# lh3/miniasm

Measured on NVIDIA H100. Metric: paf_overlaps_per_sec_ingest_to_gfa, higher is better.
Workload: dtype int64/uint32 (+3 float32 predicates)

## Files before the change

miniasm_b200/csrc/ingest_dev.cu:

```cuda
#include "ingest_dev.cuh"
#include "shard_comm.cuh"
#include <cub/cub.cuh>

struct PLine {
	uint32_t ql, qs, qe, tl, ts, te, ml_rev, bl;
	uint32_t tdelta;
	uint32_t qnl, tnl;
	uint32_t nf;
};

struct __align__(16) PRec {
	uint32_t qs, qe, ts, te;
	uint32_t ml_rev;
	uint32_t bl_f;
	uint32_t slot_q, slot_t;
};
static_assert(sizeof(PRec) == 32, "PRec layout");
constexpr uint32_t NOSLOT = 0xffffffffu;

constexpr int NL_THREADS = 256;
constexpr int NL_PER_THREAD = 4;
constexpr uint64_t NL_TILE = (uint64_t)NL_THREADS * NL_PER_THREAD * 16;

__device__ __forceinline__ uint32_t nl_mask4(uint32_t w) { return __vcmpeq4(w, 0x0a0a0a0au); }

__device__ __forceinline__ uint32_t nl_bits16(const char *text, size_t len, uint64_t off)
{
	if (off >= len) return 0;
	uint32_t bits = 0;
	if (off + 16 <= len) {
		const uint4 w = __ldg(reinterpret_cast<const uint4*>(text + off));
		const uint32_t m[4] = { nl_mask4(w.x), nl_mask4(w.y), nl_mask4(w.z), nl_mask4(w.w) };
		#pragma unroll
		for (int k = 0; k < 4; ++k) bits |= ((m[k] & 1) | (m[k] >> 7 & 2) | (m[k] >> 14 & 4) | (m[k] >> 21 & 8)) << (4 * k);
	} else for (uint64_t k = 0; off + k < len; ++k) bits |= (uint32_t)(text[off + k] == '\n') << k;
	if (off + 16 >= len && len - 1 - off < 16) bits &= ~(1u << (len - 1 - off));
	return bits;
}

__global__ void __launch_bounds__(NL_THREADS) k_nl_count(const char *__restrict__ text, size_t len, uint64_t n_tile, uint64_t *cnt)
{
	typedef cub::BlockReduce<uint32_t, NL_THREADS> BR;
	__shared__ typename BR::TempStorage ts;
	for (uint64_t t = blockIdx.x; t < n_tile; t += gridDim.x) {
		uint32_t c = 0;
		#pragma unroll
		for (int k = 0; k < NL_PER_THREAD; ++k) c += __popc(nl_bits16(text, len, t * NL_TILE + ((uint64_t)k * NL_THREADS + threadIdx.x) * 16));
		c = BR(ts).Sum(c);
		if (threadIdx.x == 0) cnt[t] = c;
		__syncthreads();
	}
	if (blockIdx.x == 0 && threadIdx.x == 0) cnt[n_tile] = 0;
}

__global__ void __launch_bounds__(NL_THREADS) k_nl_write(const char *__restrict__ text, size_t len, uint64_t n_tile, const uint64_t *__restrict__ base, uint64_t *out)
{
	typedef cub::BlockScan<uint32_t, NL_THREADS> BS;
	__shared__ typename BS::TempStorage ts;
	for (uint64_t t = blockIdx.x; t < n_tile; t += gridDim.x) {
		uint64_t at = base[t];
		#pragma unroll
		for (int k = 0; k < NL_PER_THREAD; ++k) {
			const uint64_t off = t * NL_TILE + ((uint64_t)k * NL_THREADS + threadIdx.x) * 16;
			uint32_t bits = nl_bits16(text, len, off), rank, total;
			BS(ts).ExclusiveSum((uint32_t)__popc(bits), rank, total);
			uint64_t *o = out + at + rank;
			while (bits) { const int b = __ffs(bits) - 1; *o++ = off + b + 1; bits &= bits - 1; }
			at += total;
			__syncthreads();
		}
	}
}

__host__ __device__ __forceinline__ uint32_t field_to_u32(const char *p, const char *e)
{
	while (p < e && (*p == ' ' || (*p >= '\t' && *p <= '\r'))) ++p;
	bool neg = false;
	if (p < e && (*p == '-' || *p == '+')) neg = *p == '-', ++p;
	while (p < e && *p == '0') ++p;
	unsigned long long v = 0;
	int nd = 0;
	for (; p < e; ++p, ++nd) {
		const unsigned dgt = (unsigned)(*p - '0');
		if (dgt > 9) break;
		if (nd < 18) { v = v * 10 + dgt; continue; }
// ... 33 lines not shown
{
	const uint32_t len = (uint32_t)(e - p);
	uint32_t nt = 0;
	{
		const uintptr_t a = (uintptr_t)p & ~(uintptr_t)3;
		const int lead = (int)((uintptr_t)p - a);
		for (int off = -lead; off < (int)len && nt < 11; off += 4) {
			uint32_t bits = tab_bits4(*reinterpret_cast<const uint32_t*>(p + off));
			while (bits) {
#ifdef __CUDA_ARCH__
				const int pos = off + __ffs(bits) - 1;
#else
				const int pos = off + __builtin_ctz(bits);
#endif
				bits &= bits - 1;
				if (pos >= 0 && pos < (int)len && nt < 11) tab[nt++ * 32] = (uint32_t)pos;
			}
		}
	}
	const uint32_t nf = nt + 1 < 11 ? nt + 1 : 11;
	#define COL_S(k) ((k) ? tab[((k) - 1) * 32] + 1 : 0u)
	#define COL_T(k) ((uint32_t)(k) < nt ? tab[(k) * 32] : len)
	memset(&r, 0, sizeof(r));
	r.nf = nf;
	r.qnl = COL_T(0);
	if (nf > 1) r.ql = num_field(p, COL_S(1), COL_T(1));
	if (nf > 2) r.qs = num_field(p, COL_S(2), COL_T(2));
	if (nf > 3) r.qe = num_field(p, COL_S(3), COL_T(3));
	if (nf > 4) { const uint32_t s4 = COL_S(4); r.ml_rev = (COL_T(4) > s4 && p[s4] == '-') ? 0x80000000u : 0; }
	if (nf > 5) {
		const uint32_t s5 = COL_S(5), t5 = COL_T(5);
		r.tnl = t5 - s5, r.tdelta = s5;
	}
	if (nf > 6) r.tl = num_field(p, COL_S(6), COL_T(6));
	if (nf > 7) r.ts = num_field(p, COL_S(7), COL_T(7));
	if (nf > 8) r.te = num_field(p, COL_S(8), COL_T(8));
	if (nf > 9) r.ml_rev |= num_field(p, COL_S(9), COL_T(9)) & 0x7fffffffu;
	if (nf > 10) r.bl = num_field(p, COL_S(10), COL_T(10));
	#undef COL_S
	#undef COL_T
}

struct NameTab {
	unsigned long long *key;
	unsigned long long *first;
	uint32_t *id;
	uint64_t mask;
	uint32_t *hits = nullptr;
};
constexpr int NT_OFF_BITS = 37;
constexpr unsigned long long NT_OFF_MASK = (1ull << NT_OFF_BITS) - 1;

__device__ __forceinline__ uint32_t tab_insert(const NameTab &t, const char *__restrict__ text, const char *nm, uint32_t nl, uint64_t goff, uint64_t occ,
                                               unsigned long long *overflow)
{
	const uint64_t h = name_hash(nm, 0, nl, 0);
	const unsigned long long mine = (h >> 37) << NT_OFF_BITS | (goff + 1);
	uint64_t s = h & t.mask;
	for (int probe = 0; probe < 1 << 14; ++probe, s = (s + 1) & t.mask) {
		unsigned long long k = t.key[s];
		if (k == 0) {
			k = atomicCAS(&t.key[s], 0ull, mine);
			if (k == 0) k = mine;
		}
		if ((k ^ mine) >> NT_OFF_BITS) continue;
		bool same = k == mine;
		if (!same) {
			const char *w = text + ((k & NT_OFF_MASK) - 1);
			same = true;
			for (uint32_t i = 0; same && i < nl; ++i) same = w[i] == nm[i];
			same = same && w[nl] == '\t';
		}
		if (!same) continue;
		if (t.first[s] > occ) atomicMin(&t.first[s], (unsigned long long)occ);
		return (uint32_t)s;
	}
	atomicAdd(overflow, 1ull);
	return 0;
}

constexpr int PT_THREADS = 128;
constexpr uint32_t PT_TILE = 8192;
constexpr uint32_t PT_OVER = 1024;
constexpr uint32_t PT_LIST = 1024;
static_assert(PT_TILE == PT_THREADS * 64, "each thread scans 64 bytes of its tile for line starts");
static_assert(PT_OVER % 16 == 0 && PT_OVER <= PT_TILE, "the overhang ends inside the tile after the parsed ones");

typedef cub::ScanTileState<unsigned long long> LineTileState;
typedef cub::TilePrefixCallbackOp<unsigned long long, ::cuda::std::plus<unsigned long long>, LineTileState> LinePrefixOp;

enum { PC_PARSED = 0, PC_STORED, PC_OVERFLOW, PC_LINES, PC_CUT, PC_N };

__device__ __forceinline__ uint32_t nl_bits_u4(const uint4 w)
{
	const uint32_t m[4] = { nl_mask4(w.x), nl_mask4(w.y), nl_mask4(w.z), nl_mask4(w.w) };
	uint32_t bits = 0;
	#pragma unroll
	for (int k = 0; k < 4; ++k) bits |= ((m[k] & 1) | (m[k] >> 7 & 2) | (m[k] >> 14 & 4) | (m[k] >> 21 & 8)) << (4 * k);
	return bits;
}

__global__ void k_tiles_init(LineTileState ts, int n_tile) { ts.InitializeStatus(n_tile); }

template <class P>
__global__ void __launch_bounds__(PT_THREADS)
k_parse_tiles(const char *__restrict__ text, size_t len, size_t avail, uint64_t t_lo, uint64_t line_cap, unsigned *tile_ctr, LineTileState tstate,
              int min_span, int min_match, int bi_dir, P pol)
{
	typedef cub::BlockScan<uint32_t, PT_THREADS> BS;
	__shared__ __align__(16) char s_text[PT_TILE + PT_OVER + 16];
	__shared__ uint16_t s_start[PT_LIST + 1];
	__shared__ uint32_t s_vals[PT_THREADS / 32][11][32];
	__shared__ typename BS::TempStorage s_scan;
	__shared__ typename LinePrefixOp::TempStorage s_pref;
	__shared__ unsigned long long s_first, s_tile, s_eol;
	__shared__ uint32_t s_nl;
	const uint32_t lane = threadIdx.x & 31;
	if (threadIdx.x == 0) s_tile = t_lo + atomicAdd(tile_ctr, 1u), s_nl = ~0u;
	__syncthreads();
	const uint64_t t = s_tile, b0 = t * PT_TILE, b1 = b0 + PT_TILE < len ? b0 + PT_TILE : len;
	const uint64_t w_end = b1 + PT_OVER < avail ? b1 + PT_OVER : avail;
	{
		const uint32_t n16 = (uint32_t)((w_end - b0 + 15) >> 4);
		for (uint32_t k = threadIdx.x; k < n16; k += PT_THREADS)
			reinterpret_cast<uint4*>(s_text)[k] = __ldg(reinterpret_cast<const uint4*>(text + b0) + k);
	}
	__syncthreads();
	const uint32_t my0 = threadIdx.x * 64, lim = (uint32_t)((b1 == len ? len - 1 : b1) - b0);
	uint64_t bits = 0;
	#pragma unroll
	for (int k = 0; k < 4; ++k) bits |= (uint64_t)nl_bits_u4(reinterpret_cast<const uint4*>(s_text + my0)[k]) << (16 * k);
	bits &= lim <= my0 ? 0ull : lim - my0 >= 64 ? ~0ull : (1ull << (lim - my0)) - 1;
	const bool line0 = t == 0 && threadIdx.x == 0;
	uint32_t rank, n;
	BS(s_scan).ExclusiveSum((uint32_t)__popcll(bits) + line0, rank, n);
	for (uint32_t o = lim + threadIdx.x; o < (uint32_t)(w_end - b0); o += PT_THREADS)
		if (s_text[o] == '\n' && b0 + o < len) { atomicMin(&s_nl, o); break; }
	if (threadIdx.x < 32) {
		if (t == 0) {
			if (threadIdx.x == 0) tstate.SetInclusive(0, n), s_first = 0;
		} else {
			LinePrefixOp op(tstate, s_pref, ::cuda::std::plus<unsigned long long>(), (int)t);
			const unsigned long long ex = op(n);
			if (threadIdx.x == 0) s_first = ex;
		}
	}
	__syncthreads();
	const uint64_t first = pol.line_base() + s_first;
	if (threadIdx.x == 0 && b1 == len) pol.lines_end(first + n);
	if (n == 0) return;
	uint64_t last_eol = s_nl != ~0u ? b0 + s_nl : w_end >= len ? len : ~0ull;
	if (last_eol == ~0ull) {
		if (threadIdx.x < 32) {
			uint64_t e = ~0ull;
			for (uint64_t p = w_end; p < avail; p += 32 * 16) {
				const uint64_t q = p + 16 * lane;
				uint32_t m = 0;
				for (uint32_t k = 0; k < 16 && q + k < avail; ++k) m |= (uint32_t)(text[q + k] == '\n') << k;
				const unsigned hit = __ballot_sync(0xffffffffu, m != 0);
				if (hit) { e = __shfl_sync(0xffffffffu, q + __ffs(m) - 1, __ffs(hit) - 1); break; }
			}
			if (e == ~0ull && avail == len) e = len;
			if (threadIdx.x == 0) {
				s_eol = e;
				if (e == ~0ull) pol.cut();
			}
		}
		__syncthreads();
		last_eol = s_eol;
	}
	unsigned n_parsed = 0, n_pass = 0;
	for (uint32_t r0 = 0; r0 < n; r0 += PT_LIST) {
		{
			uint32_t r = rank;
			uint64_t b = bits;
			if (line0) { if (r == r0) s_start[0] = 0; ++r; }
			for (; b && r <= r0 + PT_LIST; ++r, b &= b - 1)
				if (r >= r0) s_start[r - r0] = (uint16_t)(my0 + __ffsll((long long)b));
		}
		__syncthreads();
		const uint32_t cnt = n - r0 < PT_LIST ? n - r0 : PT_LIST;
		for (uint32_t j0 = 0; j0 < cnt; j0 += PT_THREADS) {
			const uint32_t j = j0 + threadIdx.x;
			const uint64_t i = first + r0 + j;
			uint32_t sq = NOSLOT, st = 0;
			if (j < cnt && i < line_cap) {
				const uint64_t s = b0 + s_start[j];
				uint64_t eol = r0 + j + 1 < n ? b0 + s_start[j + 1] - 1 : last_eol;
				if (eol != ~0ull) {
					const char *base = eol <= w_end ? s_text - b0 : text;
					if (eol - s > 1 && base[eol - 1] == '\r') --eol;
					PLine r;
					parse_line(base + s, base + eol, r, &s_vals[threadIdx.x >> 5][0][lane]);
					bool stored = false;
					if (r.nf >= 10) {
						++n_parsed;
						stored = !(r.qe - r.qs < (uint32_t)min_span || r.te - r.ts < (uint32_t)min_span || (int)(r.ml_rev & 0x7fffffffu) < min_match);
						n_pass += stored;
					}
					pol.line(text, base, s, i, r, stored, bi_dir, sq, st);
				}
			}
			if (uint32_t *hits = pol.hits()) {
				const unsigned grp = __match_any_sync(0xffffffffu, sq);
				if (sq != NOSLOT && lane == (uint32_t)__ffs(grp) - 1) atomicAdd(&hits[sq], (uint32_t)__popc(grp));
				if (sq != NOSLOT && bi_dir && st != sq) atomicAdd(&hits[st], 1u);
			}
		}
		__syncthreads();
	}
	pol.flush(lane, __reduce_add_sync(0xffffffffu, n_parsed), __reduce_add_sync(0xffffffffu, n_pass));
}

struct ParseStore {
	NameTab tab;
	PRec *out;
	uint64_t *start;
	unsigned long long *counts;

	__device__ __forceinline__ uint64_t line_base() const { return 0; }
	__device__ __forceinline__ void lines_end(uint64_t n) const { counts[PC_LINES] = n; }
	__device__ __forceinline__ void cut() const { atomicAdd(counts + PC_CUT, 1ull); }
	__device__ __forceinline__ uint32_t *hits() const { return tab.hits; }
	__device__ __forceinline__ void line(const char *text, const char *base, uint64_t s, uint64_t i, const PLine &r, bool stored, int, uint32_t &sq, uint32_t &st)
	{
		if (stored) {
			sq = tab_insert(tab, text, base + s, r.qnl, s, 2 * i, counts + PC_OVERFLOW);
			st = tab_insert(tab, text, base + s + r.tdelta, r.tnl, s + r.tdelta, 2 * i + 1, counts + PC_OVERFLOW);
		}
		start[i] = s;
		*reinterpret_cast<uint4*>(out + i) = make_uint4(r.qs, r.qe, r.ts, r.te);
		*(reinterpret_cast<uint4*>(out + i) + 1) = make_uint4(r.ml_rev, (r.bl & 0x7fffffffu) | (r.nf >= 11 ? 0x80000000u : 0u), sq, st);
	}
	__device__ __forceinline__ void flush(uint32_t lane, unsigned n_parsed, unsigned n_pass) const
	{
		if (lane == 0) {
			if (n_parsed) atomicAdd(counts + PC_PARSED, (unsigned long long)n_parsed);
			if (n_pass) atomicAdd(counts + PC_STORED, (unsigned long long)n_pass);
		}
	}
};

__device__ __forceinline__ uint32_t line_bl(const PRec *ln, uint64_t i, uint32_t carry_bl)
{
	if (ln[i].bl_f >> 31) return ln[i].bl_f & 0x7fffffffu;
	for (uint64_t j = i; j-- > 0;)
		if (ln[j].bl_f >> 31) return ln[j].bl_f & 0x7fffffffu;
	return carry_bl & 0x7fffffffu;
}

struct SlotUsed {
	const unsigned long long *first;
	__device__ __forceinline__ bool operator()(uint64_t s) const { return first[s] != ~0ull; }
};

__device__ __forceinline__ void occ_name(const char *text, const uint64_t *start, uint64_t occ, uint64_t *noff, uint32_t *nlen, uint32_t *slen)
{
	const char *p = text + start[occ >> 1];
	uint64_t q = 0;
	if (occ & 1) { int tabs = 0; while (tabs < 5) tabs += p[q++] == '\t'; }
	uint64_t e = q;
	while (p[e] != '\t') ++e;
	*noff = start[occ >> 1] + q, *nlen = (uint32_t)(e - q);
	uint64_t f = e + 1;
	while (p[f] != '\t') ++f;
	*slen = field_to_u32(p + e + 1, p + f);
}

__global__ void k_nocont_mark(const PRec *ln, uint64_t n_lines, const char *text, const uint64_t *start, int max_hang, float int_frac, uint8_t *excl)
{
	for (uint64_t i = blockIdx.x * (uint64_t)blockDim.x + threadIdx.x; i < n_lines; i += (uint64_t)gridDim.x * blockDim.x) {
		const PRec r = ln[i];
		if (r.slot_q == NOSLOT) continue;
		uint64_t no; uint32_t nl, ql, tl;
		occ_name(text, start, 2 * i, &no, &nl, &ql);
		occ_name(text, start, 2 * i + 1, &no, &nl, &tl);
		const bool rev = r.ml_rev >> 31;
		const int l5 = (int)(rev ? tl - r.te : r.ts), l3 = (int)(rev ? r.ts : tl - r.te);
		if (ql >> 1 > tl) {
			if (l5 > max_hang >> 2 || l3 > max_hang >> 2 || (float)(r.te - r.ts) < __fmul_rn((float)tl, int_frac)) continue;
			if ((int)r.qs - l5 > max_hang << 1 && (int)(ql - r.qe) - l3 > max_hang << 1) excl[r.slot_t] = 1;
		} else if (ql < tl >> 1) {
			if (r.qs > (uint32_t)(max_hang >> 2) || ql - r.qe > (uint32_t)(max_hang >> 2) || (float)(r.qe - r.qs) < __fmul_rn((float)ql, int_frac)) continue;
			if (l5 - (int)r.qs > max_hang << 1 && l3 - (int)(ql - r.qe) > max_hang << 1) excl[r.slot_q] = 1;
		}
	}
}

__global__ void k_nocont_drop(PRec *ln, uint64_t n_lines, const uint8_t *excl, int bi_dir, NameTab t)
{
	for (uint64_t i = blockIdx.x * (uint64_t)blockDim.x + threadIdx.x; i < n_lines; i += (uint64_t)gridDim.x * blockDim.x) {
		const uint32_t sq = ln[i].slot_q, st = ln[i].slot_t;
		if (sq == NOSLOT) continue;
// ... 126 lines not shown
	void *tmp = d.tmp(tb);
	cub::DeviceRadixSort::SortPairs(tmp, tb, dk, dv, (int)n, lo_bit, hi_bit, d.stream);
	++d.n_lib;
	d.zero_scal(SC_AUX, 1);
	rank(dk.Current(), dv.Current(), n, d.d_scal + SC_AUX);
	const unsigned long long tot_len = d.get_scal(SC_AUX);
	d.free(fa); d.free(fb); d.free(sb);
	return tot_len;
}

template <class Rank>
static void rank_reads(MabDev &d, const NameTab &tab, uint64_t cap, int lo_bit, int hi_bit, Rank rank, DHits &h, DNames &names, IngestStats &st,
                       uint32_t *&cur, uint32_t *&bfirst)
{
	uint64_t *slots = mab_alloc<uint64_t>(d, cap);
	const uint32_t n_seq = names_alloc(d, names, list_slots(d, cap, SlotUsed{tab.first}, slots));
	uint32_t *read_cnt = mab_alloc<uint32_t>(d, (size_t)n_seq + 1), *first = mab_alloc<uint32_t>(d, (size_t)n_seq + 1);
	MAB_CUDA(cudaMemsetAsync(read_cnt + n_seq, 0, 4, d.stream));
	st.tot_len = rank_slots(d, slots, n_seq, tab.first, lo_bit, hi_bit,
	                        [&](const unsigned long long *fs, const uint64_t *ss, uint32_t n, unsigned long long *tot) { rank(fs, ss, n, tot, read_cnt); });
	d.free(slots);
	d.trace("ingest:rank_ids");
	dh_bucket_first(d, read_cnt, n_seq, first);
	MAB_CUDA(cudaMemsetAsync(read_cnt, 0, (size_t)n_seq * 4, d.stream));
	uint32_t n_hits;
	MAB_CUDA(cudaMemcpyAsync(&n_hits, first + n_seq, 4, cudaMemcpyDeviceToHost, d.stream));
	d.sync();
	dh_reserve(d, h, n_hits ? n_hits : 1);
	h.n = n_hits, h.n_seq = n_seq;
	st.n_hits = n_hits, st.n_seq = n_seq;
	cur = read_cnt, bfirst = first;
}

static NameTab tab_alloc(MabDev &d, uint64_t cap, bool with_hits)
{
	NameTab tab;
	tab.key = (unsigned long long*)mab_alloc<uint64_t>(d, cap);
	tab.first = (unsigned long long*)mab_alloc<uint64_t>(d, cap);
	tab.id = mab_alloc<uint32_t>(d, cap);
	tab.mask = cap - 1;
	MAB_CUDA(cudaMemsetAsync(tab.key, 0, cap * 8, d.stream));
	MAB_CUDA(cudaMemsetAsync(tab.first, 0xff, cap * 8, d.stream));
	if (with_hits) {
		tab.hits = mab_alloc<uint32_t>(d, cap);
		MAB_CUDA(cudaMemsetAsync(tab.hits, 0, cap * 4, d.stream));
	}
	return tab;
}

static void tab_free(MabDev &d, NameTab &t)
{
	d.free(t.key); d.free(t.first); d.free(t.id);
	if (t.hits) d.free(t.hits);
	t = NameTab{nullptr, nullptr, nullptr, 0};
}

struct Parsed {
	uint64_t *start = nullptr;
	PRec *ln = nullptr;
	NameTab tab{nullptr, nullptr, nullptr, 0};
	uint64_t cap = 0, n_lines = 0, n_parsed = 0;
	uint32_t regrow = 0;
};

static inline uint64_t line_estimate(size_t len) { return len / 24 + 1024; }
static inline uint64_t tab_cap_for(uint64_t line_cap) { uint64_t cap = 1ull << 20; while (cap < line_cap / 8) cap <<= 1; return cap; }

static LineTileState tiles_alloc(MabDev &d, uint64_t n_tile, void **mem)
{
	if (n_tile >= (1ull << 31) - 64) { fprintf(stderr, "[E::miniasm_b200] more than 2^31 tiles of PAF on one GPU\n"); exit(73); }
	size_t bytes = 0;
	MAB_CUDA(LineTileState::AllocationSize((int)n_tile, bytes));
	*mem = d.alloc(bytes);
	LineTileState ts;
	MAB_CUDA(ts.Init((int)n_tile, *mem, bytes));
	return ts;
}

static void tiles_reset(MabDev &d, LineTileState ts, uint64_t n_tile)
{
	MAB_LAUNCH(d, k_tiles_init, mab_grid(n_tile, 256, 1u << 30), 256, 0, ts, (int)n_tile);
}

static void parse_resident(MabDev &d, const char *d_text, size_t len, int min_span, int min_match, int bi_dir, bool count_hits, Parsed &p)
{
	const uint64_t n_tile = (len + PT_TILE - 1) / PT_TILE;
	uint64_t line_cap = line_estimate(len), cap = tab_cap_for(line_cap);
	unsigned *ctr = mab_alloc<unsigned>(d, 1);
	void *ts_mem = nullptr;
	const LineTileState ts = tiles_alloc(d, n_tile, &ts_mem);
	for (;;) {
		p.start = mab_alloc<uint64_t>(d, line_cap);
		p.ln = mab_alloc<PRec>(d, line_cap);
		p.tab = tab_alloc(d, cap, count_hits);
		d.zero_scal(SC_COUNT, PC_N);
		if (n_tile) {
			tiles_reset(d, ts, n_tile);
			MAB_CUDA(cudaMemsetAsync(ctr, 0, 4, d.stream));
			MAB_LAUNCH(d, k_parse_tiles<ParseStore>, (unsigned)n_tile, PT_THREADS, 0, d_text, len, len, 0, line_cap, ctr, ts, min_span, min_match, bi_dir,
			           ParseStore{p.tab, p.ln, p.start, d.d_scal + SC_COUNT});
		}
		p.n_parsed = d.get_scal(SC_COUNT + PC_PARSED);
		p.n_lines = d.h_scal[SC_COUNT + PC_LINES];
		const bool more_lines = p.n_lines > line_cap, overflow = d.h_scal[SC_COUNT + PC_OVERFLOW] != 0;
		if (!more_lines && !overflow) break;
		d.free(p.start); d.free(p.ln); tab_free(d, p.tab);
		if (more_lines) line_cap = p.n_lines;
		if (overflow) cap <<= 2, ++p.regrow;
		if (cap > (1ull << 33)) { fprintf(stderr, "[E::miniasm_b200] read-name table overflow\n"); exit(77); }
	}
	d.free(ctr); d.free(ts_mem);
	p.cap = cap;
}

static void ingest_finish(MabDev &d, const char *d_text, size_t len, uint64_t *start, PRec *ln, uint64_t n_lines, NameTab tab, uint64_t cap, int bi_dir,
                          const NoContParams *nocont, DHits &h, DNames &names, IngestStats &st);

void ingest_paf(MabDev &d, const char *d_text, size_t len, int min_span, int min_match, int bi_dir, DHits &h, DNames &names, IngestStats &st,
                const NoContParams *nocont)
{
	ingest_open(len, h, names, st);
	if (len == 0) { dh_reserve(d, h, 1); return; }

	d.trace("ingest:begin");
	Parsed p;
	parse_resident(d, d_text, len, min_span, min_match, bi_dir, true, p);
	st.n_parsed = p.n_parsed, st.n_lines = p.n_lines, st.name_regrow = p.regrow;
	d.trace("ingest:parse");
	ingest_finish(d, d_text, len, p.start, p.ln, p.n_lines, p.tab, p.cap, bi_dir, nocont, h, names, st);
}

static bool stream_parse(MabDev &d, char *d_text, const char *host_text, size_t len, int min_span, int min_match, int bi_dir, bool count_hits, Parsed &p)
{
	const uint64_t CH_TILES = (64ull << 20) / PT_TILE, n_tile = (len + PT_TILE - 1) / PT_TILE;
	const uint64_t n_chunk = (n_tile + CH_TILES - 1) / CH_TILES;
	const uint64_t line_cap = line_estimate(len), cap = tab_cap_for(line_cap);
	p.start = mab_alloc<uint64_t>(d, line_cap);
	p.ln = mab_alloc<PRec>(d, line_cap);
	p.tab = tab_alloc(d, cap, count_hits);
	unsigned *ctr = mab_alloc<unsigned>(d, n_chunk);
	MAB_CUDA(cudaMemsetAsync(ctr, 0, n_chunk * 4, d.stream));
	void *ts_mem = nullptr;
	const LineTileState ts = tiles_alloc(d, n_tile, &ts_mem);
	tiles_reset(d, ts, n_tile);
	d.zero_scal(SC_COUNT, PC_N);
	if (!d.copy_stream) MAB_CUDA(cudaStreamCreateWithFlags(&d.copy_stream, cudaStreamNonBlocking));
	std::vector<cudaEvent_t> ev(n_chunk);
	cudaEvent_t ready;
	MAB_CUDA(cudaEventCreateWithFlags(&ready, cudaEventDisableTiming));
	MAB_CUDA(cudaEventRecord(ready, d.stream));
	MAB_CUDA(cudaStreamWaitEvent(d.copy_stream, ready, 0));
	uint64_t t_done = 0;
	for (uint64_t k = 0; k < n_chunk; ++k) {
		const uint64_t t0 = k * CH_TILES, t1 = (k + 1) * CH_TILES < n_tile ? (k + 1) * CH_TILES : n_tile;
		const uint64_t b0 = t0 * PT_TILE, b1 = t1 * PT_TILE < len ? t1 * PT_TILE : len;
		MAB_CUDA(cudaEventCreateWithFlags(&ev[k], cudaEventDisableTiming));
		MAB_CUDA(cudaMemcpyAsync(d_text + b0, host_text + b0, b1 - b0, cudaMemcpyHostToDevice, d.copy_stream));
		MAB_CUDA(cudaEventRecord(ev[k], d.copy_stream));
		MAB_CUDA(cudaStreamWaitEvent(d.stream, ev[k], 0));
		const uint64_t t_hi = k + 1 == n_chunk ? n_tile : t1 - 1;
		MAB_LAUNCH(d, k_parse_tiles<ParseStore>, (unsigned)(t_hi - t_done), PT_THREADS, 0, d_text, len, b1, t_done, line_cap, ctr + k, ts, min_span, min_match,
		           bi_dir, ParseStore{p.tab, p.ln, p.start, d.d_scal + SC_COUNT});
		t_done = t_hi;
	}
	p.n_parsed = d.get_scal(SC_COUNT + PC_PARSED);
	for (uint64_t k = 0; k < n_chunk; ++k) MAB_CUDA(cudaEventDestroy(ev[k]));
	MAB_CUDA(cudaEventDestroy(ready));
	d.free(ctr); d.free(ts_mem);
	p.n_lines = d.h_scal[SC_COUNT + PC_LINES];
	if (p.n_lines > line_cap || d.h_scal[SC_COUNT + PC_OVERFLOW] != 0 || d.h_scal[SC_COUNT + PC_CUT] != 0) {
		d.free(p.start); d.free(p.ln); tab_free(d, p.tab);
		p = Parsed();
		return false;
	}
	p.cap = cap;
	return true;
}

void ingest_paf_stream(MabDev &d, char *d_text, const char *host_text, size_t len, int min_span, int min_match, int bi_dir,
                       DHits &h, DNames &names, IngestStats &st)
{
	ingest_open(len, h, names, st);
	if (len == 0) { dh_reserve(d, h, 1); return; }
	Parsed p;
	if (!stream_parse(d, d_text, host_text, len, min_span, min_match, bi_dir, true, p)) {
		ingest_paf(d, d_text, len, min_span, min_match, bi_dir, h, names, st, nullptr);
		++st.name_regrow;
		return;
	}
	st.n_parsed = p.n_parsed, st.n_lines = p.n_lines;
	d.trace("ingest:stream (copy + parse + dictionary + hit counts)");
	ingest_finish(d, d_text, len, p.start, p.ln, p.n_lines, p.tab, p.cap, bi_dir, nullptr, h, names, st);
}

static void ingest_finish(MabDev &d, const char *d_text, size_t len, uint64_t *start, PRec *ln, uint64_t n_lines, NameTab tab, uint64_t cap, int bi_dir,
                          const NoContParams *nocont, DHits &h, DNames &names, IngestStats &st)
{
	if (2 * n_lines >= (1ull << 32)) { fprintf(stderr, "[E::miniasm_b200] more than 2^31 PAF lines on one GPU\n"); exit(73); }
	d.trace("ingest:dictionary");
	if (nocont) {
		uint8_t *excl = mab_alloc<uint8_t>(d, cap);
		MAB_CUDA(cudaMemsetAsync(excl, 0, cap, d.stream));
		MAB_LAUNCH(d, k_nocont_mark, mab_grid(n_lines, 256), 256, 0, ln, n_lines, d_text, start, nocont->max_hang, nocont->int_frac, excl);
		d.zero_scal(SC_AUX, 1);
		MAB_LAUNCH(d, k_count_u8, mab_grid(cap, 256), 256, 0, excl, cap, d.d_scal + SC_AUX);
		MAB_CUDA(cudaMemsetAsync(tab.first, 0xff, cap * 8, d.stream));
		MAB_CUDA(cudaMemsetAsync(tab.hits, 0, cap * 4, d.stream));
		MAB_LAUNCH(d, k_nocont_drop, mab_grid(n_lines, 256), 256, 0, ln, n_lines, excl, bi_dir, tab);
		st.n_dropped = d.get_scal(SC_AUX);
		d.free(excl);
		d.trace("ingest:-R prefilter");
	}
	uint32_t *read_cnt, *first;
	rank_reads(d, tab, cap, 0, (int)bits_for(2 * n_lines + 1), [&](const unsigned long long *fs, const uint64_t *ss, uint32_t n, unsigned long long *tot, uint32_t *cnt) {
		MAB_LAUNCH(d, k_dict_rank, mab_grid(n, 256), 256, 0, fs, ss, n, tab, d_text, start, names.off, names.nlen, names.slen, tot, cnt);
	}, h, names, st, read_cnt, first);
	if (h.n) MAB_LAUNCH(d, k_hit_emit, mab_grid(n_lines, 256), 256, 0, ln, n_lines, bi_dir, tab, first, read_cnt, h.a2);
	d.free(ln); d.free(start);
	tab_free(d, tab);

	d.trace("ingest:emit_hits");
	dh_sort_buckets(d, h, first);
	d.free(read_cnt); d.free(first);
	d.trace("ingest:sort_hits");
}

extern "C" int mab_test_parse_line(const char *line, size_t len, uint32_t *out)
{
	static uint32_t vals[11 * 32];
	PLine r;
	size_t eol = len;
	if (eol > 1 && line[eol - 1] == '\r') --eol;
	parse_line(line, line + eol, r, vals);
	out[0] = r.nf, out[1] = r.ql, out[2] = r.qs, out[3] = r.qe, out[4] = r.ml_rev >> 31, out[5] = r.tl, out[6] = r.ts, out[7] = r.te;
	out[8] = r.ml_rev & 0x7fffffffu, out[9] = r.bl, out[10] = r.qnl, out[11] = r.tnl, out[12] = r.tdelta;
	return 0;
}

__global__ void k_last_bl(const PRec *ln, uint64_t n_lines, unsigned long long *out)
{
	unsigned long long mx = 0;
	for (uint64_t i = blockIdx.x * (uint64_t)blockDim.x + threadIdx.x; i < n_lines; i += (uint64_t)gridDim.x * blockDim.x)
		if (ln[i].bl_f >> 31) mx = i + 1;
	#pragma unroll
	for (int o = 16; o; o >>= 1) { unsigned long long t = __shfl_xor_sync(0xffffffffu, mx, o); mx = t > mx ? t : mx; }
// ... 614 lines not shown
	unsigned long long s = BR(ts).Sum(sum);
	if (threadIdx.x == 0 && s) atomicAdd(tot_len, s);
}

__global__ void k_last_nl(const char *p, uint64_t n, unsigned long long *out)
{
	unsigned long long best = 0;
	for (uint64_t i = blockIdx.x * (uint64_t)blockDim.x + threadIdx.x; i < n; i += (uint64_t)gridDim.x * blockDim.x) if (p[i] == '\n') best = i + 1;
	typedef cub::BlockReduce<unsigned long long, 256> BR;
	__shared__ typename BR::TempStorage t;
	best = BR(t).Reduce(best, cub::Max());
	if (threadIdx.x == 0 && best) atomicMax(out, best);
}

struct WinRun {
	MabDev &d;
	const TextSource &src;
	size_t cap;
	char *host[2] = {nullptr, nullptr}, *dev[2] = {nullptr, nullptr};
	cudaEvent_t copied[2], parsed[2];
	void *ts_mem = nullptr;
	LineTileState ts;
	unsigned *ctr = nullptr;
	unsigned long long *ws = nullptr, *nl = nullptr;

	WinRun(MabDev &dev_, const TextSource &s, size_t w) : d(dev_), src(s), cap(0)
	{
		for (int i = 0; i < 2; ++i) {
			MAB_CUDA(cudaEventCreateWithFlags(&copied[i], cudaEventDisableTiming));
			MAB_CUDA(cudaEventCreateWithFlags(&parsed[i], cudaEventDisableTiming));
		}
		ctr = mab_alloc<unsigned>(d, 1);
		ws = (unsigned long long*)mab_alloc<uint64_t>(d, WS_N);
		nl = (unsigned long long*)mab_alloc<uint64_t>(d, 1);
		if (!d.copy_stream) MAB_CUDA(cudaStreamCreateWithFlags(&d.copy_stream, cudaStreamNonBlocking));
		resize(w, 0, 0);
	}
	~WinRun()
	{
		d.sync();
		MAB_CUDA(cudaStreamSynchronize(d.copy_stream));
		for (int i = 0; i < 2; ++i) {
			if (host[i]) MAB_CUDA(cudaFreeHost(host[i]));
			d.free(dev[i]);
			MAB_CUDA(cudaEventDestroy(copied[i])); MAB_CUDA(cudaEventDestroy(parsed[i]));
		}
		d.free(ts_mem); d.free(ctr); d.free(ws); d.free(nl);
	}
	void resize(size_t w, int b, size_t keep)
	{
		if (cap) { d.sync(); MAB_CUDA(cudaStreamSynchronize(d.copy_stream)); }
		for (int i = 0; i < 2; ++i) {
			if (!src.fill) {
				char *nh;
				MAB_CUDA(cudaMallocHost(&nh, w));
				if (i == b && keep) memcpy(nh, host[i], keep);
				if (host[i]) MAB_CUDA(cudaFreeHost(host[i]));
				host[i] = nh;
			}
			char *old = dev[i];
			if (!(src.fill && i == b && keep) && old) d.free(old), old = nullptr;
			dev[i] = (char*)d.alloc(w + 64);
			if (old) { MAB_CUDA(cudaMemcpyAsync(dev[i], old, keep, cudaMemcpyDeviceToDevice, d.stream)); d.free(old); }
		}
		if (ts_mem) d.free(ts_mem);
		ts = tiles_alloc(d, w / PT_TILE + 1, &ts_mem);
		cap = w;
	}
	void check_offsets(uint64_t store_cap) const
	{
		if (store_cap + cap >= (1ull << NT_OFF_BITS) - 1) { fprintf(stderr, "[E::miniasm_b200] more than 2^37 bytes of read names and window\n"); exit(73); }
	}
	void grow(int b, size_t keep, uint64_t store_cap)
	{
		resize(2 * cap, b, keep);
		check_offsets(store_cap);
	}
	template <int PASS>
	void launch(int b, size_t cut, int min_span, int min_match, int bi_dir, const WinParse<PASS> &pol)
	{
		const uint64_t n_tile = (cut + PT_TILE - 1) / PT_TILE;
		tiles_reset(d, ts, n_tile);
		MAB_CUDA(cudaMemsetAsync(ctr, 0, 4, d.stream));
		MAB_LAUNCH(d, k_parse_tiles<WinParse<PASS>>, (unsigned)n_tile, PT_THREADS, 0, dev[b], cut, cut, 0, ~0ull, ctr, ts, min_span, min_match, bi_dir, pol);
		MAB_CUDA(cudaMemcpyAsync(ws + WS_LINE_IN, ws + WS_LINE_OUT, 16, cudaMemcpyDeviceToDevice, d.stream));
		MAB_CUDA(cudaEventRecord(parsed[b], d.stream));
	}
};

template <int PASS>
static bool win_pass(WinRun &w, int min_span, int min_match, int bi_dir, const WinTab &tab, const uint32_t *bfirst, uint32_t *cur, DHit *out, uint64_t *n_bytes)
{
	MabDev &d = w.d;
	if (w.src.rewind(w.src.ud) != 0) return false;
	w.check_offsets(tab.store_cap);
	MAB_CUDA(cudaMemsetAsync(w.ws, 0, WS_N * 8, d.stream));
	const WinParse<PASS> pol{tab, w.ws, bfirst, cur, out};
	cudaEvent_t ready;
	MAB_CUDA(cudaEventCreateWithFlags(&ready, cudaEventDisableTiming));
	MAB_CUDA(cudaEventRecord(ready, d.stream));
	MAB_CUDA(cudaStreamWaitEvent(d.copy_stream, ready, 0));
	const char *tail = nullptr;
	size_t n_tail = 0, total = 0;
	bool eof = false;
	if (w.src.fill) {
		size_t tail_at = 0;
		for (int b = 0; !eof; b ^= 1) {
			if (n_tail) MAB_CUDA(cudaMemcpyAsync(w.dev[b], w.dev[b ^ 1] + tail_at, n_tail, cudaMemcpyDeviceToDevice, d.stream));
			size_t have = n_tail, cut = 0;
			for (;;) {
				while (have < w.cap) {
					const int64_t r = w.src.fill(w.src.ud, w.dev[b] + have, w.cap - have);
					if (r == TS_FULL) break;
					if (r < 0) {
						if (PASS == 2) { fprintf(stderr, "[E::miniasm_b200] the PAF source failed when read again after %llu bytes\n", (unsigned long long)total); exit(78); }
						d.sync();
						MAB_CUDA(cudaEventDestroy(ready));
						return false;
					}
					if (r == 0) { eof = true; break; }
					have += (size_t)r, total += (size_t)r;
				}
				if (eof) { cut = have; break; }
				if (have) {
					MAB_CUDA(cudaMemsetAsync(w.nl, 0, 8, d.stream));
					const size_t look = have < (1u << 20) ? have : (1u << 20);
					MAB_LAUNCH(d, k_last_nl, mab_grid(look, 256), 256, 0, w.dev[b] + (have - look), (uint64_t)look, w.nl);
					unsigned long long nl = 0;
					MAB_CUDA(cudaMemcpyAsync(&nl, w.nl, 8, cudaMemcpyDeviceToHost, d.stream));
					d.sync();
					if (nl) nl += have - look;
					else if (look < have) {
						MAB_LAUNCH(d, k_last_nl, mab_grid(have - look, 256), 256, 0, w.dev[b], (uint64_t)(have - look), w.nl);
						MAB_CUDA(cudaMemcpyAsync(&nl, w.nl, 8, cudaMemcpyDeviceToHost, d.stream));
						d.sync();
					}
					if (nl) { cut = (size_t)nl; break; }
				}
				w.grow(b, have, tab.store_cap);
			}
			tail_at = cut, n_tail = have - cut;
			if (cut == 0) break;
			w.launch(b, cut, min_span, min_match, bi_dir, pol);
		}
	}
	for (int b = 0; !eof; b ^= 1) {
		MAB_CUDA(cudaEventSynchronize(w.copied[b]));
		if (n_tail) memcpy(w.host[b], tail, n_tail);
		size_t have = n_tail, cut = 0;
		for (;;) {
			while (have < w.cap) {
				const size_t r = w.src.read(w.src.ud, w.host[b] + have, w.cap - have);
				if (r == 0) { eof = true; break; }
				have += r, total += r;
			}
			if (eof) { cut = have; break; }
			const char *nl = (const char*)memrchr(w.host[b], '\n', have);
			if (nl) { cut = (size_t)(nl - w.host[b]) + 1; break; }
			w.grow(b, have, tab.store_cap);
		}
		tail = w.host[b] + cut, n_tail = have - cut;
		if (cut == 0) break;
		MAB_CUDA(cudaStreamWaitEvent(d.copy_stream, w.parsed[b], 0));
		MAB_CUDA(cudaMemcpyAsync(w.dev[b], w.host[b], cut, cudaMemcpyHostToDevice, d.copy_stream));
		MAB_CUDA(cudaEventRecord(w.copied[b], d.copy_stream));
		MAB_CUDA(cudaStreamWaitEvent(d.stream, w.copied[b], 0));
		w.launch(b, cut, min_span, min_match, bi_dir, pol);
// ... 70 lines not shown
```

Before: 1.668 billion.

## Make tile parser persistent with async double-buffered loads and cross-tile line queue

The tile-parsing kernel becomes persistent: a grid sized to occupancy claims tiles in a loop and prefetches the next tile into a second shared buffer with cp.async while the current one is parsed. Line starts go into a shared ring queue shared across tiles, so parse rounds always run with full 128-thread occupancy instead of leaving threads idle on short tail batches. The aim is to hide global load latency and cut idle lanes and launch overhead. In exchange the kernel uses double the text shared memory and carries more complex queue and index bookkeeping. The decoupled-lookback chain also now runs inside persistent blocks, which can stall when tiles are claimed out of order.

```diff
diff --git a/miniasm_b200/csrc/ingest_dev.cu b/miniasm_b200/csrc/ingest_dev.cu
--- a/miniasm_b200/csrc/ingest_dev.cu
+++ b/miniasm_b200/csrc/ingest_dev.cu
@@ -1,6 +1,7 @@
 #include "ingest_dev.cuh"
 #include "shard_comm.cuh"
 #include <cub/cub.cuh>
+#include <cuda_pipeline.h>
 
 struct PLine {
 	uint32_t ql, qs, qe, tl, ts, te, ml_rev, bl;
@@ -200,9 +201,13 @@
 constexpr int PT_THREADS = 128;
 constexpr uint32_t PT_TILE = 8192;
 constexpr uint32_t PT_OVER = 1024;
-constexpr uint32_t PT_LIST = 1024;
+constexpr uint32_t PT_LIST = 128;
+constexpr uint32_t PT_RING = 256;
+constexpr uint16_t PT_LAST = 0x4000, PT_BUF = 0x8000;
 static_assert(PT_TILE == PT_THREADS * 64, "each thread scans 64 bytes of its tile for line starts");
 static_assert(PT_OVER % 16 == 0 && PT_OVER <= PT_TILE, "the overhang ends inside the tile after the parsed ones");
+static_assert(PT_THREADS - 1 + PT_LIST + 1 <= PT_RING && (PT_RING & (PT_RING - 1)) == 0, "the queue ring holds a remainder and a list");
+static_assert(PT_TILE <= PT_LAST, "line starts fit below the flag bits of a queue entry");
 
 typedef cub::ScanTileState<unsigned long long> LineTileState;
 typedef cub::TilePrefixCallbackOp<unsigned long long, ::cuda::std::plus<unsigned long long>, LineTileState> LinePrefixOp;
@@ -221,112 +226,146 @@
 __global__ void k_tiles_init(LineTileState ts, int n_tile) { ts.InitializeStatus(n_tile); }
 
 template <class P>
-__global__ void __launch_bounds__(PT_THREADS)
-k_parse_tiles(const char *__restrict__ text, size_t len, size_t avail, uint64_t t_lo, uint64_t line_cap, unsigned *tile_ctr, LineTileState tstate,
-              int min_span, int min_match, int bi_dir, P pol)
-{
-	typedef cub::BlockScan<uint32_t, PT_THREADS> BS;
-	__shared__ __align__(16) char s_text[PT_TILE + PT_OVER + 16];
-	__shared__ uint16_t s_start[PT_LIST + 1];
+__global__ void __launch_bounds__(PT_THREADS, 9)
+k_parse_tiles(const char *__restrict__ text, size_t len, size_t avail, uint64_t t_lo, uint64_t t_hi, uint64_t line_cap, unsigned *tile_ctr,
+              LineTileState tstate, int min_span, int min_match, int bi_dir, P pol)
+{
+	typedef cub::BlockScan<uint32_t, PT_THREADS, cub::BLOCK_SCAN_WARP_SCANS> BS;
+	__shared__ __align__(16) char s_text[2][PT_TILE + PT_OVER + 16];
+	__shared__ uint16_t s_q[PT_RING];
 	__shared__ uint32_t s_vals[PT_THREADS / 32][11][32];
 	__shared__ typename BS::TempStorage s_scan;
 	__shared__ typename LinePrefixOp::TempStorage s_pref;
-	__shared__ unsigned long long s_first, s_tile, s_eol;
+	__shared__ unsigned long long s_b0[2], s_wend[2], s_leol[2];
+	__shared__ unsigned long long s_first, s_tile, s_ia;
 	__shared__ uint32_t s_nl;
 	const uint32_t lane = threadIdx.x & 31;
-	if (threadIdx.x == 0) s_tile = t_lo + atomicAdd(tile_ctr, 1u), s_nl = ~0u;
-	__syncthreads();
-	const uint64_t t = s_tile, b0 = t * PT_TILE, b1 = b0 + PT_TILE < len ? b0 + PT_TILE : len;
-	const uint64_t w_end = b1 + PT_OVER < avail ? b1 + PT_OVER : avail;
-	{
-		const uint32_t n16 = (uint32_t)((w_end - b0 + 15) >> 4);
-		for (uint32_t k = threadIdx.x; k < n16; k += PT_THREADS)
-			reinterpret_cast<uint4*>(s_text)[k] = __ldg(reinterpret_cast<const uint4*>(text + b0) + k);
-	}
-	__syncthreads();
-	const uint32_t my0 = threadIdx.x * 64, lim = (uint32_t)((b1 == len ? len - 1 : b1) - b0);
-	uint64_t bits = 0;
-	#pragma unroll
-	for (int k = 0; k < 4; ++k) bits |= (uint64_t)nl_bits_u4(reinterpret_cast<const uint4*>(s_text + my0)[k]) << (16 * k);
-	bits &= lim <= my0 ? 0ull : lim - my0 >= 64 ? ~0ull : (1ull << (lim - my0)) - 1;
-	const bool line0 = t == 0 && threadIdx.x == 0;
-	uint32_t rank, n;
-	BS(s_scan).ExclusiveSum((uint32_t)__popcll(bits) + line0, rank, n);
-	for (uint32_t o = lim + threadIdx.x; o < (uint32_t)(w_end - b0); o += PT_THREADS)
-		if (s_text[o] == '\n' && b0 + o < len) { atomicMin(&s_nl, o); break; }
-	if (threadIdx.x < 32) {
-		if (t == 0) {
-			if (threadIdx.x == 0) tstate.SetInclusive(0, n), s_first = 0;
-		} else {
-			LinePrefixOp op(tstate, s_pref, ::cuda::std::plus<unsigned long long>(), (int)t);
-			const unsigned long long ex = op(n);
-			if (threadIdx.x == 0) s_first = ex;
-		}
-	}
-	__syncthreads();
-	const uint64_t first = pol.line_base() + s_first;
-	if (threadIdx.x == 0 && b1 == len) pol.lines_end(first + n);
-	if (n == 0) return;
-	uint64_t last_eol = s_nl != ~0u ? b0 + s_nl : w_end >= len ? len : ~0ull;
-	if (last_eol == ~0ull) {
+
+	auto claim = [&](int b) {
+		if (threadIdx.x == 0) s_tile = t_lo + atomicAdd(tile_ctr, 1u);
+		__syncthreads();
+		const uint64_t t = s_tile;
+		if (t < t_hi) {
+			const uint64_t b0 = t * PT_TILE, b1 = b0 + PT_TILE < len ? b0 + PT_TILE : len;
+			const uint64_t w_end = b1 + PT_OVER < avail ? b1 + PT_OVER : avail;
+			const uint32_t n16 = (uint32_t)((w_end - b0 + 15) >> 4);
+			for (uint32_t k = threadIdx.x; k < n16; k += PT_THREADS) __pipeline_memcpy_async(s_text[b] + 16 * k, text + b0 + 16 * k, 16);
+			if (threadIdx.x == 0) s_b0[b] = b0, s_wend[b] = w_end;
+		}
+		__pipeline_commit();
+	};
+
+	uint32_t head = 0, qn = 0, qa = 0;
+	uint64_t ib = 0;
+	unsigned n_parsed = 0, n_pass = 0;
+	auto round = [&](uint32_t m) {
+		const uint32_t j = threadIdx.x;
+		const uint64_t i = j < qa ? s_ia + j : ib + (j - qa);
+		uint32_t sq = NOSLOT, st = 0;
+		if (j < m && i < line_cap) {
+			const uint16_t q = s_q[(head + j) & (PT_RING - 1)];
+			const int b = q & PT_BUF ? 1 : 0;
+			const uint64_t b0 = s_b0[b], s = b0 + (q & (PT_LAST - 1));
+			uint64_t eol = q & PT_LAST ? s_leol[b] : b0 + (s_q[(head + j + 1) & (PT_RING - 1)] & (PT_LAST - 1)) - 1;
+			if (eol != ~0ull) {
+				const char *base = eol <= s_wend[b] ? s_text[b] - b0 : text;
+				if (eol - s > 1 && base[eol - 1] == '\r') --eol;
+				PLine r;
+				parse_line(base + s, base + eol, r, &s_vals[threadIdx.x >> 5][0][lane]);
+				bool stored = false;
+				if (r.nf >= 10) {
+					++n_parsed;
+					stored = !(r.qe - r.qs < (uint32_t)min_span || r.te - r.ts < (uint32_t)min_span || (int)(r.ml_rev & 0x7fffffffu) < min_match);
+					n_pass += stored;
+				}
+				pol.line(text, base, s, i, r, stored, bi_dir, sq, st);
+			}
+		}
+		if (uint32_t *hits = pol.hits()) {
+			const unsigned grp = __match_any_sync(0xffffffffu, sq);
+			if (sq != NOSLOT && lane == (uint32_t)__ffs(grp) - 1) atomicAdd(&hits[sq], (uint32_t)__popc(grp));
+			if (sq != NOSLOT && bi_dir && st != sq) atomicAdd(&hits[st], 1u);
+		}
+		__syncthreads();
+		head += m, qn -= m, ib += m - qa, qa = 0;
+	};
+
+	int cb = 0;
+	claim(cb);
+	if (s_tile >= t_hi) return;
+	for (;;) {
+		const uint64_t t = s_tile;
+		if (threadIdx.x == 0) s_nl = ~0u;
+		__pipeline_wait_prior(0);
+		__syncthreads();
+		const char *tx = s_text[cb];
+		const uint64_t b0 = t * PT_TILE, b1 = b0 + PT_TILE < len ? b0 + PT_TILE : len;
+		const uint64_t w_end = b1 + PT_OVER < avail ? b1 + PT_OVER : avail;
+		const uint32_t my0 = threadIdx.x * 64, lim = (uint32_t)((b1 == len ? len - 1 : b1) - b0);
+		uint64_t bits = 0;
+		#pragma unroll
+		for (int k = 0; k < 4; ++k) bits |= (uint64_t)nl_bits_u4(reinterpret_cast<const uint4*>(tx + my0)[k]) << (16 * k);
+		bits &= lim <= my0 ? 0ull : lim - my0 >= 64 ? ~0ull : (1ull << (lim - my0)) - 1;
+		const bool line0 = t == 0 && threadIdx.x == 0;
+		uint32_t rank, n;
+		BS(s_scan).ExclusiveSum((uint32_t)__popcll(bits) + line0, rank, n);
+		for (uint32_t o = lim + threadIdx.x; o < (uint32_t)(w_end - b0); o += PT_THREADS)
+			if (tx[o] == '\n' && b0 + o < len) { atomicMin(&s_nl, o); break; }
 		if (threadIdx.x < 32) {
-			uint64_t e = ~0ull;
-			for (uint64_t p = w_end; p < avail; p += 32 * 16) {
-				const uint64_t q = p + 16 * lane;
-				uint32_t m = 0;
-				for (uint32_t k = 0; k < 16 && q + k < avail; ++k) m |= (uint32_t)(text[q + k] == '\n') << k;
-				const unsigned hit = __ballot_sync(0xffffffffu, m != 0);
-				if (hit) { e = __shfl_sync(0xffffffffu, q + __ffs(m) - 1, __ffs(hit) - 1); break; }
+			if (t == 0) {
+				if (threadIdx.x == 0) tstate.SetInclusive(0, n), s_first = 0;
+			} else {
+				LinePrefixOp op(tstate, s_pref, ::cuda::std::plus<unsigned long long>(), (int)t);
+				const unsigned long long ex = op(n);
+				if (threadIdx.x == 0) s_first = ex;
 			}
-			if (e == ~0ull && avail == len) e = len;
-			if (threadIdx.x == 0) {
-				s_eol = e;
-				if (e == ~0ull) pol.cut();
+		}
+		if (threadIdx.x == 0) s_ia = ib;
+		__syncthreads();
+		const uint64_t first = pol.line_base() + s_first;
+		if (threadIdx.x == 0 && b1 == len) pol.lines_end(first + n);
+		qa = qn, ib = first;
+		if (n) {
+			uint64_t last_eol = s_nl != ~0u ? b0 + s_nl : w_end >= len ? len : ~0ull;
+			if (last_eol == ~0ull) {
+				if (threadIdx.x < 32) {
+					uint64_t e = ~0ull;
+					for (uint64_t p = w_end; p < avail; p += 32 * 16) {
+						const uint64_t q = p + 16 * lane;
+						uint32_t m = 0;
+						for (uint32_t k = 0; k < 16 && q + k < avail; ++k) m |= (uint32_t)(text[q + k] == '\n') << k;
+						const unsigned hit = __ballot_sync(0xffffffffu, m != 0);
+						if (hit) { e = __shfl_sync(0xffffffffu, q + __ffs(m) - 1, __ffs(hit) - 1); break; }
+					}
+					if (e == ~0ull && avail == len) e = len;
+					if (threadIdx.x == 0) {
+						s_leol[cb] = e;
+						if (e == ~0ull) pol.cut();
+					}
+				}
+			} else if (threadIdx.x == 0) s_leol[cb] = last_eol;
+			const uint16_t buf = cb ? PT_BUF : 0;
+			for (uint32_t r0 = 0; r0 < n; r0 += PT_LIST) {
+				const uint32_t cnt = n - r0 < PT_LIST ? n - r0 : PT_LIST;
+				{
+					const uint32_t at = head + qn - r0;
+					uint32_t r = rank;
+					uint64_t b = bits;
+					if (line0) { if (r == r0) s_q[at & (PT_RING - 1)] = buf | (n == 1 ? PT_LAST : 0); ++r; }
+					for (; b && r <= r0 + cnt; ++r, b &= b - 1)
+						if (r >= r0) s_q[(at + r) & (PT_RING - 1)] = buf | (r + 1 == n ? PT_LAST : 0) | (uint16_t)(my0 + __ffsll((long long)b));
+				}
+				__syncthreads();
+				qn += cnt;
+				if (qn >= PT_THREADS) round(PT_THREADS);
 			}
 		}
-		__syncthreads();
-		last_eol = s_eol;
-	}
-	unsigned n_parsed = 0, n_pass = 0;
-	for (uint32_t r0 = 0; r0 < n; r0 += PT_LIST) {
-		{
-			uint32_t r = rank;
-			uint64_t b = bits;
-			if (line0) { if (r == r0) s_start[0] = 0; ++r; }
-			for (; b && r <= r0 + PT_LIST; ++r, b &= b - 1)
-				if (r >= r0) s_start[r - r0] = (uint16_t)(my0 + __ffsll((long long)b));
-		}
-		__syncthreads();
-		const uint32_t cnt = n - r0 < PT_LIST ? n - r0 : PT_LIST;
-		for (uint32_t j0 = 0; j0 < cnt; j0 += PT_THREADS) {
-			const uint32_t j = j0 + threadIdx.x;
-			const uint64_t i = first + r0 + j;
-			uint32_t sq = NOSLOT, st = 0;
-			if (j < cnt && i < line_cap) {
-				const uint64_t s = b0 + s_start[j];
-				uint64_t eol = r0 + j + 1 < n ? b0 + s_start[j + 1] - 1 : last_eol;
-				if (eol != ~0ull) {
-					const char *base = eol <= w_end ? s_text - b0 : text;
-					if (eol - s > 1 && base[eol - 1] == '\r') --eol;
-					PLine r;
-					parse_line(base + s, base + eol, r, &s_vals[threadIdx.x >> 5][0][lane]);
-					bool stored = false;
-					if (r.nf >= 10) {
-						++n_parsed;
-						stored = !(r.qe - r.qs < (uint32_t)min_span || r.te - r.ts < (uint32_t)min_span || (int)(r.ml_rev & 0x7fffffffu) < min_match);
-						n_pass += stored;
-					}
-					pol.line(text, base, s, i, r, stored, bi_dir, sq, st);
-				}
-			}
-			if (uint32_t *hits = pol.hits()) {
-				const unsigned grp = __match_any_sync(0xffffffffu, sq);
-				if (sq != NOSLOT && lane == (uint32_t)__ffs(grp) - 1) atomicAdd(&hits[sq], (uint32_t)__popc(grp));
-				if (sq != NOSLOT && bi_dir && st != sq) atomicAdd(&hits[st], 1u);
-			}
-		}
-		__syncthreads();
-	}
+		if (qa) round(qn);
+		claim(cb ^ 1);
+		if (s_tile >= t_hi) break;
+		cb ^= 1;
+	}
+	if (qn) round(qn);
 	pol.flush(lane, __reduce_add_sync(0xffffffffu, n_parsed), __reduce_add_sync(0xffffffffu, n_pass));
 }
 
@@ -619,6 +658,22 @@
 	MAB_LAUNCH(d, k_tiles_init, mab_grid(n_tile, 256, 1u << 30), 256, 0, ts, (int)n_tile);
 }
 
+template <class P>
+static unsigned parse_grid(uint64_t n_tile)
+{
+	static const unsigned fit = [] {
+		int dev = 0, sms = 0, per_sm = 0;
+		MAB_CUDA(cudaGetDevice(&dev));
+		MAB_CUDA(cudaDeviceGetAttribute(&sms, cudaDevAttrMultiProcessorCount, dev));
+		MAB_CUDA(cudaOccupancyMaxActiveBlocksPerMultiprocessor(&per_sm, k_parse_tiles<P>, PT_THREADS, 0));
+		unsigned g = (unsigned)(sms * (per_sm > 0 ? per_sm : 1));
+		const char *e = getenv("MAB_PARSE_CTAS");
+		if (e && atoi(e) > 0 && (unsigned)atoi(e) < g) g = (unsigned)atoi(e);
+		return g;
+	}();
+	return n_tile < fit ? (unsigned)(n_tile ? n_tile : 1) : fit;
+}
+
 static void parse_resident(MabDev &d, const char *d_text, size_t len, int min_span, int min_match, int bi_dir, bool count_hits, Parsed &p)
 {
 	const uint64_t n_tile = (len + PT_TILE - 1) / PT_TILE;
@@ -634,8 +689,8 @@
 		if (n_tile) {
 			tiles_reset(d, ts, n_tile);
 			MAB_CUDA(cudaMemsetAsync(ctr, 0, 4, d.stream));
-			MAB_LAUNCH(d, k_parse_tiles<ParseStore>, (unsigned)n_tile, PT_THREADS, 0, d_text, len, len, 0, line_cap, ctr, ts, min_span, min_match, bi_dir,
-			           ParseStore{p.tab, p.ln, p.start, d.d_scal + SC_COUNT});
+			MAB_LAUNCH(d, k_parse_tiles<ParseStore>, parse_grid<ParseStore>(n_tile), PT_THREADS, 0, d_text, len, len, 0, n_tile, line_cap, ctr, ts,
+			           min_span, min_match, bi_dir, ParseStore{p.tab, p.ln, p.start, d.d_scal + SC_COUNT});
 		}
 		p.n_parsed = d.get_scal(SC_COUNT + PC_PARSED);
 		p.n_lines = d.h_scal[SC_COUNT + PC_LINES];
@@ -696,8 +751,8 @@
 		MAB_CUDA(cudaEventRecord(ev[k], d.copy_stream));
 		MAB_CUDA(cudaStreamWaitEvent(d.stream, ev[k], 0));
 		const uint64_t t_hi = k + 1 == n_chunk ? n_tile : t1 - 1;
-		MAB_LAUNCH(d, k_parse_tiles<ParseStore>, (unsigned)(t_hi - t_done), PT_THREADS, 0, d_text, len, b1, t_done, line_cap, ctr + k, ts, min_span, min_match,
-		           bi_dir, ParseStore{p.tab, p.ln, p.start, d.d_scal + SC_COUNT});
+		MAB_LAUNCH(d, k_parse_tiles<ParseStore>, parse_grid<ParseStore>(t_hi - t_done), PT_THREADS, 0, d_text, len, b1, t_done, t_hi, line_cap, ctr + k, ts,
+		           min_span, min_match, bi_dir, ParseStore{p.tab, p.ln, p.start, d.d_scal + SC_COUNT});
 		t_done = t_hi;
 	}
 	p.n_parsed = d.get_scal(SC_COUNT + PC_PARSED);
@@ -1478,7 +1533,8 @@
 		const uint64_t n_tile = (cut + PT_TILE - 1) / PT_TILE;
 		tiles_reset(d, ts, n_tile);
 		MAB_CUDA(cudaMemsetAsync(ctr, 0, 4, d.stream));
-		MAB_LAUNCH(d, k_parse_tiles<WinParse<PASS>>, (unsigned)n_tile, PT_THREADS, 0, dev[b], cut, cut, 0, ~0ull, ctr, ts, min_span, min_match, bi_dir, pol);
+		MAB_LAUNCH(d, k_parse_tiles<WinParse<PASS>>, parse_grid<WinParse<PASS>>(n_tile), PT_THREADS, 0, dev[b], cut, cut, 0, n_tile, ~0ull, ctr, ts, min_span,
+		           min_match, bi_dir, pol);
 		MAB_CUDA(cudaMemcpyAsync(ws + WS_LINE_IN, ws + WS_LINE_OUT, 16, cudaMemcpyDeviceToDevice, d.stream));
 		MAB_CUDA(cudaEventRecord(parsed[b], d.stream));
 	}
```

Result: no change. 1.662 billion, median of 6 (-0.3%).
